# JSybrandt/HypergraphEmbedding

Measured on AMD Instinct MI355X. Metric: training samples/sec + alg-dist SpMV GB/s, HOBE dim=128 at 1/2/4/8 MI355X, higher is better.
Workload: dtype f32; 1 GPU; C3 HG2V_ALG_DIST (HOBE) dim=128, random 100k/50k, 1 step = 1 training epoch; nodes=100000, edges=50000, nnz=1999903, records_per_epoch=59999992, batch=256, dim=128, num_neighbors=5, num_samples=200, parallelism=single GPU

## Files before the change

hypergraphembedding_amd/csrc/hgx_ctx.hip:

```cpp
#include <algorithm>
#include <cstring>
#include <vector>

#include "hgx_internal.h"

int hgx_fail(hgx_ctx *ctx, int code, const char *fmt, ...) {
  if (ctx) {
    char buf[1024];
    va_list ap;
    va_start(ap, fmt);
    vsnprintf(buf, sizeof(buf), fmt, ap);
    va_end(ap);
    ctx->err = buf;
  }
  return code;
}

int hgx_ensure(hgx_ctx *ctx, DevBuf &b, size_t bytes) {
  if (bytes == 0) bytes = 16;
  if (b.bytes >= bytes) return HGX_OK;
  if (b.p) {
    hipFree(b.p);
    b.p = nullptr;
    b.bytes = 0;
// ... 34 lines not shown
    delete ctx;
    return HGX_EHIP;
  }
  ctx->stream = ctx->own_stream;
  hipEventCreate(&ctx->ev0);
  hipEventCreate(&ctx->ev1);
  *out = ctx;
  return HGX_OK;
}

extern "C" int hgx_destroy(hgx_ctx *ctx) {
  if (!ctx) return HGX_OK;
  hipSetDevice(ctx->device);
  hipStreamSynchronize(ctx->stream);
  DevBuf *bufs[] = {&ctx->rp_n, &ctx->col_n, &ctx->rp_e, &ctx->col_e,
                    &ctx->X[0], &ctx->X[1], &ctx->Y[0], &ctx->Y[1], &ctx->mm,
                    &ctx->rp_el, &ctx->col_el, &ctx->blk_n, &ctx->blk_e,
                    &ctx->blk_sn, &ctx->blk_el,
                    &ctx->rec_idx, &ctx->rec_tgt, &ctx->ntab, &ctx->etab,
                    &ctx->nacc, &ctx->eacc, &ctx->s0, &ctx->s1, &ctx->s2,
                    &ctx->s3, &ctx->s4, &ctx->s5, &ctx->s6, &ctx->s7,
                    &ctx->feat_n, &ctx->feat_e, &ctx->cn_p, &ctx->cn_j,
                    &ctx->cn_v, &ctx->ce_p, &ctx->ce_j, &ctx->ce_v,
                    &ctx->hw_n, &ctx->hw_e, &ctx->hw_self, &ctx->bloom_off, &ctx->bloom_bits, &ctx->store,
                    &ctx->st_sel, &ctx->st_keys, &ctx->st_vals, &ctx->st_tmp,
                    &ctx->st_hist};
  for (DevBuf *b : bufs) hgx_release(*b);
  for (LongRows *l : {&ctx->long_n, &ctx->long_e, &ctx->long_sn, &ctx->long_el})
    for (DevBuf *b : {&l->seg, &l->off, &l->rows, &l->part}) hgx_release(*b);
  for (LongRows &l : ctx->long_elr)
    for (DevBuf *b : {&l.seg, &l.off, &l.rows, &l.part}) hgx_release(*b);
  for (hipStream_t &s : ctx->tstream)
    if (s) hipStreamDestroy(s);
  if (ctx->ev0) hipEventDestroy(ctx->ev0);
  if (ctx->ev1) hipEventDestroy(ctx->ev1);
  if (ctx->own_stream) hipStreamDestroy(ctx->own_stream);
  delete ctx;
  return HGX_OK;
}

extern "C" const char *hgx_last_error(const hgx_ctx *ctx) {
  return ctx ? ctx->err.c_str() : "null context";
}

extern "C" int hgx_set_stream(hgx_ctx *ctx, void *hip_stream) {
  if (!ctx) return HGX_EINVAL;
  ctx->stream = hip_stream ? (hipStream_t)hip_stream : ctx->own_stream;
  return HGX_OK;
}

extern "C" int hgx_set_tuning(hgx_ctx *ctx, const char *key, int64_t value) {
  if (!ctx) return HGX_EINVAL;
  HGX_CHECK(ctx, key, HGX_EINVAL, "null tuning key");
  const std::string k(key);
  Tuning &t = ctx->tune;
  if (k == "sample_reject_w") {
    HGX_CHECK(ctx, value >= 0, HGX_EINVAL, "sample_reject_w must be >= 0");
    t.sample_reject_w = value;
  } else if (k == "sample_mode3_shift_e") {
    HGX_CHECK(ctx, value >= -10 && value <= 10, HGX_EINVAL,
              "sample_mode3_shift_e must be in [-10, 10]");
    t.sample_mode3_shift_e = (int)value;
  } else if (k == "sample_mode3_shift") {
    HGX_CHECK(ctx, value >= -10 && value <= 10, HGX_EINVAL,
              "sample_mode3_shift must be in [-10, 10]");
    t.sample_mode3_shift = (int)value;
  } else if (k == "sample_mode3") {
    HGX_CHECK(ctx, value >= 0 && value <= 2, HGX_EINVAL, "sample_mode3 must be 0, 1 or 2");
    t.sample_mode3 = (int)value;
  } else if (k == "train_fused") {
    HGX_CHECK(ctx, value == 0 || value == 1, HGX_EINVAL, "train_fused must be 0 or 1");
    t.train_fused = (int)value;
  } else if (k == "train_lanes") {
    HGX_CHECK(ctx, value == 0 || value == 32 || value == 64, HGX_EINVAL,
              "train_lanes must be 0, 32 or 64");
    t.train_lanes = (int)value;
  } else if (k == "train_tb") {
    HGX_CHECK(ctx, value == 0 || value == 128 || value == 256 || value == 512, HGX_EINVAL,
              "train_tb must be 0, 128, 256 or 512");
    t.train_tb = (int)value;
  } else if (k == "train_wave_pair") {
    HGX_CHECK(ctx, (value >= -1 && value <= 1) || value == 3, HGX_EINVAL,
              "train_wave_pair must be -1, 0, 1 or 3");
    t.train_wave_pair = (int)value;
  } else if (k == "alg_long") {
    HGX_CHECK(ctx, value == 0 || (value >= 64 && value <= (1 << 20)), HGX_EINVAL,
              "alg_long must be 0 or in [64, 2^20]");
    t.alg_long = (int)value;
  } else if (k == "alg_push") {
    HGX_CHECK(ctx, value == 0 || value == 1, HGX_EINVAL, "alg_push must be 0 or 1");
    t.alg_push = (int)value;
  } else if (k == "mlp_fuse_head") {
    HGX_CHECK(ctx, value == 0 || value == 1, HGX_EINVAL, "mlp_fuse_head must be 0 or 1");
    t.mlp_fuse_head = (int)value;
  } else if (k == "mlp_prefetch") {
    HGX_CHECK(ctx, value >= 0 && value <= 2, HGX_EINVAL, "mlp_prefetch must be 0, 1 or 2");
    t.mlp_prefetch = (int)value;
  } else if (k == "mlp_wgrad_split") {
    HGX_CHECK(ctx, value >= 0 && value <= 1, HGX_EINVAL, "mlp_wgrad_split must be 0 or 1");
    t.mlp_wgrad_split = (int)value;
  } else if (k == "svc_lds_m") {
    HGX_CHECK(ctx, value == 64 || value == 128 || value == 192, HGX_EINVAL,
              "svc_lds_m must be 64, 128 or 192");
    t.svc_lds_m = (int)value;
  } else if (k == "ae_chunk_rows") {
    HGX_CHECK(ctx, value >= 0 && value <= (1 << 16), HGX_EINVAL,
              "ae_chunk_rows must be in [0, 65536]");
    t.ae_chunk_rows = (int)value;
  } else if (k == "n2v_expand_w") {
    HGX_CHECK(ctx, value >= 0 && value <= (1 << 20), HGX_EINVAL,
              "n2v_expand_w must be in [0, 2^20]");
    t.n2v_expand_w = (int)value;
  } else if (k == "n2v_chunk_walks") {
    HGX_CHECK(ctx, value >= 0 && value <= (1 << 16), HGX_EINVAL,
              "n2v_chunk_walks must be in [0, 65536]");
    t.n2v_chunk_walks = (int)value;
// ... 200 lines not shown
```

hypergraphembedding_amd/csrc/hgx_internal.h:

```cpp
#pragma once

#include <hip/hip_runtime.h>

#include <cstdarg>
#include <cstdint>
#include <cstdio>
#include <cstdlib>
#include <string>
#include <vector>

#include "hgx.h"

struct DevBuf {
  void *p = nullptr;
  size_t bytes = 0;
  template <class T> T *as() const { return reinterpret_cast<T *>(p); }
};

struct LongRows {
  DevBuf seg;
  DevBuf off;
  DevBuf rows;
  DevBuf part;
  int nlong = 0, nseg = 0, thresh = 0;
// ... 79 lines not shown
  int K = 0;
  DevBuf rec_idx, rec_tgt;
  static constexpr int kMaxRecBlocks = 16;
  int64_t rec_bounds[kMaxRecBlocks + 1] = {0};
  int n_rec_blocks = 0;

  int smp_family = -1;
  uint64_t smp_seed = 0;
  bool rec_in_order = false;

  DevBuf store;
  int64_t n_store = 0, cap_store = 0;
  int store_family = -1, store_K = 0, store_blocks = 0;
  uint64_t store_seed = 0;
  int64_t store_carry = 0;
  std::vector<unsigned> st_hist_host;
  uint64_t st_hist_seed = 0;
  bool st_hist_ok = false;
  DevBuf st_sel, st_keys, st_vals, st_tmp, st_hist;

  int d = 0, dp = 0;
  int64_t node_rows = 0, edge_rows = 0;
  DevBuf ntab, etab, nacc, eacc;
  double train_ms = 0, train_epoch_ms = 0;
  double train_loss_sum = 0;
  int64_t train_records = 0, train_batches = 0;
  int64_t train_fused = 0, train_split = 0;
  int64_t train_multi = 0;
  int train_step_tb = 0, train_step_rpb = 0;

  DevBuf s0, s1, s2, s3, s4, s5, s6, s7;
  hipStream_t tstream[2] = {nullptr, nullptr};
  int tstream_cus = -1;
};

inline int hgx_debug_env(const char *name, int dflt) {
#ifdef HGX_DEBUG_KNOBS
  const char *e = getenv(name);
  return e && e[0] ? atoi(e) : dflt;
#else
  (void)name;
  return dflt;
#endif
}
inline const char *hgx_debug_env_str(const char *name) {
#ifdef HGX_DEBUG_KNOBS
  return getenv(name);
#else
  (void)name;
  return nullptr;
#endif
}

int hgx_fail(hgx_ctx *ctx, int code, const char *fmt, ...);
int hgx_make_row_blocks(hgx_ctx *ctx, const int32_t *rp, int32_t r0, int32_t r1,
                        DevBuf &blk, int &nblk);
int hgx_make_long_rows(hgx_ctx *ctx, const int32_t *rp, int32_t r0, int32_t r1,
                       LongRows &out);
int hgx_ensure(hgx_ctx *ctx, DevBuf &b, size_t bytes);
void hgx_release(DevBuf &b);

#define HGX_HIP(ctx, expr)                                                   \
  do {                                                                       \
    hipError_t e_ = (expr);                                                  \
    if (e_ != hipSuccess)                                                    \
      return hgx_fail((ctx), HGX_EHIP, "%s failed: %s (%s:%d)", #expr,        \
// ... 160 lines not shown
```

hypergraphembedding_amd/csrc/hgx_train.hip:

```cpp
#include <hipcub/hipcub.hpp>

#include <algorithm>
#include <cmath>
#include <cstdlib>
#include <cstring>
#include <vector>

#include "hgx_internal.h"
#include "hgx_train_common.h"
#include "hgx_train_split.h"
#include "hgx_train_step.h"
#include "hgx_train_prep.h"
#include "hgx_train_layout.h"

namespace {

int grid_for(int64_t work, int per_block) {
  int64_t g = (work + per_block - 1) / per_block;
  return (int)std::max<int64_t>(1, std::min<int64_t>(g, 4096));
}

void geometry(int d, int &L, int &VPL) {
  const int nv = (d + 3) / 4;
  L = 1;
// ... 11 lines not shown
using KFn = void (*)(TrainArgs, int);

int env_int(const char *name, int dflt) { return hgx_debug_env(name, dflt); }

template <int L, int VPL, int TB>
KFn fwd_spec(int K, int loss, int act) {
  if (K == 5 && loss == 0 && act == 0) return train_fwd_bwd<L, VPL, 5, true, 1, TB>;
  if (K == 5 && loss == 1 && act == 1) return train_fwd_bwd<L, VPL, 5, true, 2, TB>;
  return nullptr;
}

template <int L, int VPL>
KFn fwd_for(int K, int loss, int act, int tb1) {
  KFn f = tb1 == 512 ? fwd_spec<L, VPL, 512>(K, loss, act)
                     : fwd_spec<L, VPL, kTB>(K, loss, act);
  if (f) return f;
  if (K <= 2) return train_fwd_bwd<L, VPL, 2, false, 0, kTB>;
  if (K <= 5) return train_fwd_bwd<L, VPL, 5, false, 0, kTB>;
  if (K <= 8) return train_fwd_bwd<L, VPL, 8, false, 0, kTB>;
  return train_fwd_bwd<L, VPL, 16, false, 0, kTB>;
}

using KStepFn = void (*)(TrainArgs, int, int, int, int);
using KFlushFn = void (*)(TrainArgs, const int *, const int *, const int *, int, int);

template <int SL, int VW, int TB>
void step_fns(int loss, KStepFn *kf, KFlushFn &kfl) {
  kf[0] = loss == 0 ? train_step<SL, VW, 5, 1, TB, false>
                    : train_step<SL, VW, 5, 2, TB, false>;
  kf[1] = loss == 0 ? train_step<SL, VW, 5, 1, TB, true>
                    : train_step<SL, VW, 5, 2, TB, true>;
  kfl = train_flush<SL * VW / 4>;
}
template <int VW>
void step_fns_pair(int loss, KStepFn *kf, KFlushFn &kfl) {
  kf[0] = loss == 0 ? train_step<64, VW, 5, 1, 512, false, true>
                    : train_step<64, VW, 5, 2, 512, false, true>;
  kf[1] = loss == 0 ? train_step<64, VW, 5, 1, 512, true, true>
                    : train_step<64, VW, 5, 2, 512, true, true>;
  kfl = train_flush<64 * VW / 4>;
}
void step_fns_quad(int loss, KStepFn *kf, KFlushFn &kfl) {
  kf[0] = loss == 0 ? train_step_q<2, 5, 1, false, 2> : train_step_q<2, 5, 2, false, 2>;
  kf[1] = loss == 0 ? train_step_q<2, 5, 1, true, 2> : train_step_q<2, 5, 2, true, 2>;
  kfl = train_flush<32>;
}
constexpr int kPairDefault128 = 3, kPairDefault256 = 1;
bool pick_step(int L, int VPL, int K, int loss, int act, int lanes, int pair, int &sl,
               int &tb, int &rpb, KStepFn *kf, KFlushFn &kfl) {
  if (VPL != 1 || K != 5 || loss != act) return false;
  if (L != 32 && L != 64) return false;
  const int vw = L == 32 && lanes != 32 ? 2 : 4;
  sl = L * 4 / vw;
  const int pair_auto = tb != 0 ? 0 : vw == 2 ? kPairDefault128 : kPairDefault256;
  const int form = pair < 0 ? pair_auto : pair;
  if (sl == 64 && vw == 2 && form == 3) {
    tb = 512;
    rpb = 2;
    step_fns_quad(loss, kf, kfl);
    return true;
  }
  if (sl == 64 && form) {
    tb = 512;
    rpb = 4;
    if (vw == 2) step_fns_pair<2>(loss, kf, kfl);
    else step_fns_pair<4>(loss, kf, kfl);
    return true;
  }
  if (sl == 32) {
    tb = tb == 256 ? 256 : 128;
    if (tb == 128) step_fns<32, 4, 128>(loss, kf, kfl);
    else step_fns<32, 4, 256>(loss, kf, kfl);
  } else if (vw == 2) {
    tb = tb == 512 || tb == 128 ? tb : 256;
    if (tb == 512) step_fns<64, 2, 512>(loss, kf, kfl);
    else if (tb == 128) step_fns<64, 2, 128>(loss, kf, kfl);
    else step_fns<64, 2, 256>(loss, kf, kfl);
  } else {
    tb = 256;
    step_fns<64, 4, 256>(loss, kf, kfl);
  }
  rpb = tb / sl;
  return true;
}

bool pick_kernels(int L, int VPL, int K, int loss, int act, int &tb1, int tb2,
                  KFn &k1, KFn &k2) {
#define HGX_CASE(LL, VV)                                                     \
  if (L == LL && VPL == VV) {                                                \
    k1 = env_int("HGX_TRAIN_GENERIC", 0) == 1                                \
             ? train_fwd_bwd<LL, VV, 16, false, 0, kTB>                      \
             : fwd_for<LL, VV>(K, loss, act, tb1);                           \
// ... 428 lines not shown
      return HGX_OK;
    }
    hipLaunchKernelGGL(shuffle_keys, dim3(grid_for(n, 256)), dim3(256), 0, ctx->stream, seed,
                       ep, n, keys_in, vals_in);
    size_t tmp = sort_tmp;
    if (hipcub::DeviceRadixSort::SortPairs(ctx->s7.as<char>() + sort_off, tmp, keys_in, keys_out,
                                           vals_in, perm, (int)n, 0, 64, ctx->stream) != hipSuccess)
      return hgx_fail(ctx, HGX_EHIP, "shuffle sort failed");
    return HGX_OK;
  }
  int upload(const int64_t *pe) {
    hperm.resize(n);
    for (int64_t i = 0; i < n; i++) {
      if (pe[i] < 0 || pe[i] >= n)
        return hgx_fail(ctx, HGX_EINVAL, "permutation entry out of range");
      hperm[i] = (int)pe[i];
    }
    if (hipMemcpyAsync(perm, hperm.data(), sizeof(int) * n, hipMemcpyHostToDevice,
                       ctx->stream) != hipSuccess ||
        hipStreamSynchronize(ctx->stream) != hipSuccess)
      return hgx_fail(ctx, HGX_EHIP, "permutation upload failed");
    return HGX_OK;
  }
};

struct TrainRun {
  hgx_ctx *ctx;
  const TrainPlan &p;
  TrainArgs ap[2];
  int *skey[2] = {nullptr, nullptr}, *sM[2] = {nullptr, nullptr};
  double *dloss = nullptr, *dpart = nullptr;
  hipStream_t sst, spr;
  std::vector<hipEvent_t> bev, pev;
  int *hbrk = nullptr;
  hipError_t flags_err = hipSuccess;
  int64_t nfused = 0, nsplit = 0, nmulti = 0;
  double batch_ms = 0.0;

  TrainRun(hgx_ctx *c, const TrainPlan &plan) : ctx(c), p(plan), sst(c->stream), spr(c->stream) {}
  ~TrainRun() {
    for (auto e : bev) if (e) (void)hipEventDestroy(e);
    for (auto e : pev) if (e) (void)hipEventDestroy(e);
    if (hbrk) (void)hipHostFree(hbrk);
  }
  int buffers(int *perm) {
    TrainArgs &a = ap[0];
    memset(&a, 0, sizeof(a));
    const size_t s3_bytes = hgx_layout::carve_step(p, {}, a);
    const size_t s5_bytes = hgx_layout::carve_chunk(p, {}, ap, skey, sM);
    HGX_TRY(hgx_ensure(ctx, ctx->s2, sizeof(float) * (size_t)p.SB * p.dp));
    HGX_TRY(hgx_ensure(ctx, ctx->s3, s3_bytes));
    HGX_TRY(hgx_ensure(ctx, ctx->s4, sizeof(float) * (size_t)p.nbatches * p.lstride + 16));
    HGX_TRY(hgx_ensure(ctx, ctx->s5, s5_bytes));
    HGX_TRY(hgx_ensure(ctx, ctx->s6, 64 + sizeof(double) * kLossBlocks));
    HGX_HIP(ctx, hipMemsetAsync(ctx->s5.p, 0, s5_bytes, ctx->stream));
    HGX_HIP(ctx, hipMemsetAsync(ctx->s3.p, 0, s3_bytes, ctx->stream));
    a.idx = ctx->rec_idx.as<int>(), a.tgt = ctx->rec_tgt.as<float>(), a.perm = perm;
    a.n = p.n, a.B = p.batch, a.R = p.R, a.K = p.K, a.dp = p.dp;
    a.ntab = ctx->ntab.as<float>(), a.etab = ctx->etab.as<float>();
    a.nacc = ctx->nacc.as<float>(), a.eacc = ctx->eacc.as<float>();
    a.gslot = ctx->s2.as<float>(), a.lossbuf = ctx->s4.as<float>();
    a.lr = p.lr, a.eps = p.eps, a.loss = p.loss, a.act = p.act;
    a.SB = p.SB, a.nblk1 = p.nblk1, a.lstride = p.lstride;
    a.fused = p.fused ? 1 : 0, a.prpb = p.prpb, a.RW = p.RW, a.MX = p.MX, a.Mmax = p.Mmax;
    hgx_layout::carve_step(p, {ctx->s3.as<char>()}, a);
    hgx_layout::carve_chunk(p, {ctx->s5.as<char>()}, ap, skey, sM);
    dloss = reinterpret_cast<double *>(ctx->s6.as<char>() + 32);
    dpart = reinterpret_cast<double *>(ctx->s6.as<char>() + 64);
    return HGX_OK;
  }
  int init(int *perm) {
    HGX_TRY(buffers(perm));
    if (p.fused)
      HGX_HIP(ctx, hipHostMalloc(reinterpret_cast<void **>(&hbrk),
                                 sizeof(int) * p.CB * (p.overlap ? 2 : 1)));
    if (p.overlap && !p.ahead) {
      HGX_TRY(train_streams(ctx, ctx->tune.train_prep_cus));
      sst = ctx->tstream[0];
      spr = ctx->tstream[1];
    }
    bev.assign(2 * p.nchunks, nullptr);
    pev.assign(p.overlap ? p.nchunks + 1 : 0, nullptr);
    for (auto &e : bev) HGX_HIP(ctx, hipEventCreate(&e));
    for (auto &e : pev) HGX_HIP(ctx, hipEventCreateWithFlags(&e, hipEventDisableTiming));
    return HGX_OK;
  }
  int set_of(int64_t c) const { return p.overlap ? (int)(c & 1) : 0; }

  void begin_epoch() {
    (void)hipMemsetAsync(dloss, 0, sizeof(double), ctx->stream);
    (void)hipMemsetAsync(ap[0].lossbuf, 0, sizeof(float) * (size_t)p.nbatches * p.lstride,
                         ctx->stream);
    if (p.fused) (void)hipMemsetAsync(ap[0].r0acc, 0, hgx_layout::r0acc_bytes(p), ctx->stream);
    if (p.overlap && !p.ahead) {
      (void)hipEventRecord(pev[p.nchunks], ctx->stream);
      (void)hipStreamWaitEvent(sst, pev[p.nchunks], 0);
      (void)hipStreamWaitEvent(spr, pev[p.nchunks], 0);
    }
  }
  void prepare(int64_t c) {
    const int nbc = p.chunk_batches(c), cp = (int)(c & 1), set = set_of(c);
    hipLaunchKernelGGL(train_prep, dim3(p.CB), dim3(kTB), p.prep_smem, spr, ap[0], c * p.CB, nbc,
                       p.P, skey[cp], sM[cp]);
    if (!p.fused) return;
    hipLaunchKernelGGL(train_place, dim3(p.CB), dim3(kTB), p.place_smem, spr, ap[set], nbc, p.CB,
                       skey[cp], sM[cp], skey[cp ^ 1], sM[cp ^ 1], c > 0 ? 1 : 0);
    flags_err = hipMemcpyAsync(hbrk + (size_t)set * p.CB, ap[set].pbrk, sizeof(int) * nbc,
                               hipMemcpyDeviceToHost, spr);
    if (p.overlap) (void)hipEventRecord(pev[c], spr);
  }
  int wait_prepared(int64_t c) {
    hipError_t e = hipSuccess;
    if (p.overlap) {
      e = hipEventSynchronize(pev[c]);
      if (e == hipSuccess && !p.ahead) (void)hipStreamWaitEvent(sst, pev[c], 0);
    } else if (p.fused) {
      e = flags_err != hipSuccess ? flags_err : hipStreamSynchronize(spr);
    }
    if (e == hipSuccess) return HGX_OK;
    return hgx_fail(ctx, HGX_EHIP, "batch preparation failed: %s",
                    hipGetErrorString(hipGetLastError()));
  }
  void run_steps(int64_t c) {
    const int nbc = p.chunk_batches(c), set = set_of(c);
    for (int bi = 0; bi < nbc; bi++) {
      if (!p.fused) {
        hipLaunchKernelGGL(p.k1, dim3(p.nblk1), dim3(p.tb1), 0, sst, ap[0], bi);
        hipLaunchKernelGGL(p.k2, dim3(p.grid2), dim3(p.tb2), 0, sst, ap[0], bi);
        continue;
      }
      const int64_t gbat = c * p.CB + bi;
      const int nrec = (int)std::min<int64_t>(p.batch, p.n - gbat * p.batch);
      const int multi = hbrk[(size_t)set * p.CB + bi] && gbat > 0;
      nmulti += multi;
      hipLaunchKernelGGL(p.kf[multi], dim3(p.NBF), dim3(p.tbf), 0, sst, ap[set], bi, (int)gbat,
                         nrec, (int)gbat);
    }
    (p.fused ? nfused : nsplit) += nbc;
  }
  int run_chunks() {
    if (p.overlap) prepare(0);
    for (int64_t c = 0; c < p.nchunks; c++) {
      if (!p.overlap) prepare(c);
      if (p.ahead && c + 1 < p.nchunks) prepare(c + 1);
      HGX_TRY(wait_prepared(c));
      (void)hipEventRecord(bev[2 * c], sst);
      run_steps(c);
      (void)hipEventRecord(bev[2 * c + 1], sst);
      if (p.overlap && !p.ahead && c + 1 < p.nchunks) {
        if (c >= 1 && hipEventSynchronize(bev[2 * (c - 1) + 1]) != hipSuccess)
          return hgx_fail(ctx, HGX_EHIP, "batch step failed: %s",
                          hipGetErrorString(hipGetLastError()));
        prepare(c + 1);
      }
    }
    return HGX_OK;
  }
  void flush() const {
    const int cp = (int)((p.nchunks - 1) & 1), last_nbc = p.chunk_batches(p.nchunks - 1);
    const int *ml = sM[cp] + (last_nbc - 1);
    const int *mp = last_nbc >= 2 ? sM[cp] + (last_nbc - 2)
                                  : (p.nchunks >= 2 ? sM[cp ^ 1] + (p.CB - 1) : nullptr);
    const int nlast = (int)(p.n - (p.nbatches - 1) * p.batch);
    hipLaunchKernelGGL(p.kfl, dim3(64), dim3(256), 0, sst, ap[0],
                       skey[cp] + (size_t)(last_nbc - 1) * p.Mmax, ml, mp,
                       (int)(p.nbatches - 1), std::min(p.NBF, nlast));
  }
  int finish_epoch(double &lsum) {
    if (p.fused) flush();
    hipLaunchKernelGGL(loss_partial, dim3(kLossBlocks), dim3(kTB), 0, sst, ap[0].lossbuf,
                       p.nbatches * p.lstride, dpart);
    hipLaunchKernelGGL(loss_final, dim3(1), dim3(kLossBlocks), 0, sst, dpart, dloss);
    int ovf = 0;
    if (hipMemcpyAsync(&lsum, dloss, sizeof(double), hipMemcpyDeviceToHost, sst) != hipSuccess ||
        (p.fused && hipMemcpyAsync(&ovf, ap[0].ovf, sizeof(int), hipMemcpyDeviceToHost, sst) !=
                        hipSuccess) ||
        hipStreamSynchronize(sst) != hipSuccess)
      return hgx_fail(ctx, HGX_EHIP, "epoch failed: %s", hipGetErrorString(hipGetLastError()));
    if (ovf)
      return hgx_fail(ctx, HGX_ENUMERIC,
                      "a gradient left the step's fixed-point range (|g| >= %g after "
                      "the 1/batch factor, or NaN): training diverged",
                      (double)kFixLimit);
    for (int64_t c = 0; c < p.nchunks; c++) {
      float m = 0.f;
      if (hipEventElapsedTime(&m, bev[2 * c], bev[2 * c + 1]) == hipSuccess) batch_ms += m;
    }
    return HGX_OK;
  }
  float join() {
    if (p.overlap) {
      (void)hipStreamSynchronize(spr);
      (void)hipStreamSynchronize(sst);
    }
    float ms = 0.f;
    (void)hipEventRecord(ctx->ev1, ctx->stream);
    (void)hipEventSynchronize(ctx->ev1);
    (void)hipEventElapsedTime(&ms, ctx->ev0, ctx->ev1);
    return ms;
  }
  void stats(int epochs, float ms) const {
    ctx->train_ms = batch_ms;
    ctx->train_epoch_ms = ms;
    ctx->train_records = (int64_t)epochs * p.n;
    ctx->train_batches = (int64_t)epochs * p.nbatches;
    ctx->train_fused = nfused;
    ctx->train_split = nsplit;
    ctx->train_multi = nmulti;
    ctx->train_step_tb = p.fused ? p.tbf : 0;
    ctx->train_step_rpb = p.prpb;
  }
};
// ... 78 lines not shown
```

hypergraphembedding_amd/csrc/hgx_train_common.h:

```cpp
#pragma once
#include "hgx_internal.h"

namespace {

constexpr int kTB = 256;
constexpr int kChunkRound = 64;

#ifdef HGX_DEBUG_KNOBS
__constant__ int g_tab = 0;
#else
static constexpr int g_tab = 0;
#endif

#ifdef HGX_DEBUG_KNOBS
__constant__ unsigned long long *g_trace = nullptr;
__constant__ int g_trace_nb = 0;
#else
static constexpr unsigned long long *g_trace = nullptr;
static constexpr int g_trace_nb = 0;
#endif
#define HGX_STAMP(var)                                              \
  do {                                                              \
    if (g_trace) {                                                  \
      asm volatile("s_waitcnt vmcnt(0) lgkmcnt(0)" ::: "memory");   \
// ... 20 lines not shown
  int B, R, K, dp;
  float *ntab, *etab, *nacc, *eacc;
  float *gslot, *gzero, *lossbuf;
  int *bidx;
  float *btgt;
  int *inv, *ukey, *uoff, *ucount;
  int2 *bmeta;
  int SB, nblk1;
  int lstride;
  float lr, eps;
  int loss, act;
  int fused, prpb, RW, MX, Mmax;
  int *pidx, *pbrk;
  unsigned *pcode, *scode;
  float *ptgt;
  int2 *pfo;
  long long *gacc;
  float *shadow;
  long long *r0acc;
  int *ovf;
};

constexpr unsigned kSShared = 0x80000000u;
constexpr unsigned kSOwn = 0x40000000u;
constexpr unsigned kSPend = 0x20000000u;
constexpr unsigned kSLocal = 0x10000000u;
constexpr unsigned kSFirst = 0x08000000u;
constexpr unsigned kFEdge = 0x10000000u;
constexpr int kDefBits = 14;
constexpr unsigned kDefMask = 0xfffu;
constexpr unsigned kSlotMask = 0x3fffu;
constexpr int kFX = 4;
constexpr int kWX = kFX + 2;
constexpr int kPackB = 512;
constexpr int kPrepB = 1366;
constexpr int kSortP = 4096;

__device__ __forceinline__ bool slot_is_edge(int s, int K) {
  return s == 1 || s == 3 || s >= 4 + K;
}

__device__ __forceinline__ float act_f(int act, float z) {
  return act == 0 ? 1.0f / (1.0f + expf(-z)) : (z > 0.f ? z : 0.f);
}
__device__ __forceinline__ float act_d(int act, float z, float y) {
  return act == 0 ? y * (1.0f - y) : (z > 0.f ? 1.f : 0.f);
}
__device__ __forceinline__ void head_loss(int loss, float y, float yt,
                                          float &lv, float &g) {
  const float eps = 1e-7f;
  if (loss == 0) {
    const float ytc = fminf(fmaxf(yt, eps), 1.f);
    const float ypc = fminf(fmaxf(y, eps), 1.f);
    lv = ytc * logf(ytc / ypc);
    g = (y >= eps && y <= 1.f) ? -ytc / ypc : 0.f;
  } else {
    const float df = y - yt;
    lv = df * df;
    g = 2.f * df;
  }
}

__device__ __forceinline__ float4 f4(float a) { return make_float4(a, a, a, a); }
__device__ __forceinline__ float4 operator+(float4 a, float4 b) {
  return make_float4(a.x + b.x, a.y + b.y, a.z + b.z, a.w + b.w);
}
// ... 23 lines not shown
```

hypergraphembedding_amd/csrc/hgx_train_prep.h:

```cpp
#pragma once
#include <rocprim/block/block_radix_sort.hpp>

#include "hgx_train_step.h"

namespace {

__device__ int block_exclusive_scan(int v, int *total, int *s_ws) {
  const int lane = threadIdx.x & 63, wave = threadIdx.x >> 6;
  int inc = v;
#pragma unroll
  for (int off = 1; off < 64; off <<= 1) {
    const int o = __shfl_up(inc, off);
    if (lane >= off) inc += o;
  }
  if (lane == 63) s_ws[wave] = inc;
  __syncthreads();
  int base = 0, tot = 0;
  for (int w = 0; w < kTB / 64; w++) {
    if (w < wave) base += s_ws[w];
    tot += s_ws[w];
  }
  __syncthreads();
  *total = tot;
  return base + inc - v;
// ... 214 lines not shown
  const int G = (a.B + RPB - 1) / RPB * RPB;
  const int *prev = nullptr;
  int Mp = 0, Mpp = 0;
  if (cb > 0) {
    prev = skey_cur + (size_t)(cb - 1) * a.Mmax;
    Mp = sM_cur[cb - 1];
  } else if (has_prev) {
    prev = skey_pc + (size_t)(CB - 1) * a.Mmax;
    Mp = sM_pc[CB - 1];
  }
  if (cb > 1) Mpp = sM_cur[cb - 2];
  else if (has_prev) Mpp = sM_pc[CB - 2 + cb];
  const int U = a.ucount[cb];
  int *s_prev = s_dyn, *s_u = s_dyn + a.Mmax;
  __shared__ int s_brk;
  if (threadIdx.x == 0) s_brk = 0;
  for (int j = threadIdx.x; j < Mp; j += kTB) s_prev[j] = prev[j];
  for (int j = threadIdx.x; j < U; j += kTB) s_u[j] = a.ukey[(size_t)cb * SB + j];
  const int *bidx = a.bidx + (size_t)cb * a.B * R;
  const float *btgt = a.btgt + (size_t)cb * a.B * 3;
  __syncthreads();
  for (int i = threadIdx.x; i < nb && Mp; i += kTB) {
    int e0 = -1;
    for (int s2 = 0; s2 < R; s2++) {
      const int row = bidx[i * R + s2];
      if (row == 0) continue;
      const int j = bsearch_lds(s_prev, Mp, ((int)slot_is_edge(s2, K) << 30) | row);
      if (j < 0) continue;
      if (e0 >= 0 && j != e0) s_brk = 1;
      e0 = j;
    }
  }
  __syncthreads();
  if (threadIdx.x == 0) a.pbrk[cb] = s_brk;
  {
    const int per = (nb + kTB - 1) / kTB, i0 = threadIdx.x * per, i1 = min(i0 + per, nb);
    int cs = 0;
    for (int i = i0; i < i1; i++) {
      int any = 0;
      for (int s = 4; s < R; s++) any |= bidx[i * R + s];
      s_pos[i] = any;
      cs += any == 0;
    }
    int NS = 0;
    int bs = block_exclusive_scan(cs, &NS, s_ws);
    const int NBF = G / RPB;
    for (int i = i0; i < i1; i++) {
      const bool sh = s_pos[i] == 0;
      const int p = sh ? bs : NS + (i - bs);
      s_pos[i] = (p % NBF) * RPB + p / NBF;
      bs += sh;
    }
  }
  int *pidx = a.pidx + (size_t)cb * G * RW;
  unsigned *pcode = a.pcode + (size_t)cb * G * RW;
  float *ptgt = a.ptgt + (size_t)cb * G * 3;
  for (int t = threadIdx.x; t < G * RW; t += kTB) {
    pidx[t] = 0;
    pcode[t] = 0u;
  }
  for (int t = threadIdx.x; t < G * 3; t += kTB) ptgt[t] = 0.f;
  __syncthreads();
  const unsigned *sc = a.scode + (size_t)cb * SB;
  for (int t = threadIdx.x; t < nb * R; t += kTB) {
    const int i = t / R, s = t - i * R;
    const int row = bidx[t];
    unsigned code = 0;
// ... 277 lines not shown
```

hypergraphembedding_amd/csrc/hgx_train_step.h:

```cpp
#pragma once
#include "hgx_train_split.h"

namespace {



constexpr double kFixScale = 17592186044416.0;
constexpr double kFixInv = 1.0 / 17592186044416.0;
constexpr float kFixLimit = 32.f;

__device__ __forceinline__ unsigned long long to_fix(float v) {
  return (unsigned long long)__double2ll_rn((double)v * kFixScale);
}
__device__ __forceinline__ float from_fix(long long v) {
  return (float)((double)v * kFixInv);
}
__device__ __forceinline__ float act_d_nc(int act, float z, float y) {
  return act == 0 ? mul_nc(y, sub_nc(1.0f, y)) : (z > 0.f ? 1.f : 0.f);
}
__device__ __forceinline__ void head_loss_nc(int loss, float y, float yt,
                                             float &lv, float &g) {
  const float eps = 1e-7f;
  if (loss == 0) {
    const float ytc = fminf(fmaxf(yt, eps), 1.f);
    const float ypc = fminf(fmaxf(y, eps), 1.f);
    lv = mul_nc(ytc, logf(ytc / ypc));
    g = (y >= eps && y <= 1.f) ? -ytc / ypc : 0.f;
  } else {
    const float df = sub_nc(y, yt);
    lv = mul_nc(df, df);
    g = 2.f * df;
  }
}

template <int VW>
struct SV;
template <>
struct SV<4> {
  using T = float4;
  struct Fx {
    longlong2 a, b;
  };
  static __device__ __forceinline__ T zero() { return f4(0.f); }
  static __device__ __forceinline__ T add(T x, T y) { return x + y; }
  static __device__ __forceinline__ T mul(T x, float m) {
    return make_float4(x.x * m, x.y * m, x.z * m, x.w * m);
  }
  static __device__ __forceinline__ T fma(float s, T v, T c) { return fma4(s, v, c); }
  static __device__ __forceinline__ float dot(T x, T y) { return dot4(x, y); }
  static __device__ __forceinline__ void adagrad(T &p, T &ac, T g, float lr, float eps) {
    adagrad4_hw(p, ac, g, lr, eps);
  }
  static __device__ __forceinline__ void pin(T &v) {
    asm volatile("" : "+v"(v.x), "+v"(v.y), "+v"(v.z), "+v"(v.w));
  }
  static __device__ __forceinline__ Fx ldfix(const long long *e, int lane) {
    const longlong2 *g = reinterpret_cast<const longlong2 *>(e) + 2 * lane;
    return {g[0], g[1]};
  }
  static __device__ __forceinline__ T unfix(const Fx &g) {
    return make_float4(from_fix(g.a.x), from_fix(g.a.y), from_fix(g.b.x), from_fix(g.b.y));
  }
  static __device__ __forceinline__ void addfix(long long *e, int lane, T v, int &bad) {
    bad |= !(fabsf(v.x) < kFixLimit) | !(fabsf(v.y) < kFixLimit) |
           !(fabsf(v.z) < kFixLimit) | !(fabsf(v.w) < kFixLimit);
    unsigned long long *d = reinterpret_cast<unsigned long long *>(e) + 4 * lane;
    atomicAdd(d + 0, to_fix(v.x));
    atomicAdd(d + 1, to_fix(v.y));
    atomicAdd(d + 2, to_fix(v.z));
    atomicAdd(d + 3, to_fix(v.w));
  }
  static __device__ __forceinline__ void zerofix(long long *e, int lane) {
    longlong2 *g = reinterpret_cast<longlong2 *>(e) + 2 * lane;
    g[0] = g[1] = make_longlong2(0, 0);
  }
  static __device__ __forceinline__ Fx fxadd(const Fx &x, const Fx &y) {
    return {make_longlong2(x.a.x + y.a.x, x.a.y + y.a.y),
            make_longlong2(x.b.x + y.b.x, x.b.y + y.b.y)};
  }
  static __device__ __forceinline__ Fx fxzero() {
    return {make_longlong2(0, 0), make_longlong2(0, 0)};
  }
};
template <>
struct SV<2> {
  using T = float2;
  struct Fx {
    longlong2 a;
  };
  static __device__ __forceinline__ T zero() { return make_float2(0.f, 0.f); }
  static __device__ __forceinline__ T add(T x, T y) { return make_float2(x.x + y.x, x.y + y.y); }
  static __device__ __forceinline__ T mul(T x, float m) { return make_float2(x.x * m, x.y * m); }
  static __device__ __forceinline__ T fma(float s, T v, T c) {
    return make_float2(fmaf(s, v.x, c.x), fmaf(s, v.y, c.y));
  }
  static __device__ __forceinline__ float dot(T x, T y) {
    return add_nc(mul_nc(x.x, y.x), mul_nc(x.y, y.y));
  }
  static __device__ __forceinline__ void adagrad(T &p, T &ac, T g, float lr, float eps) {
    const float *gv = &g.x;
    float *pp = &p.x, *aa = &ac.x;
#pragma unroll
    for (int c = 0; c < 2; c++) {
      const float na = add_nc(aa[c], mul_nc(gv[c], gv[c]));
      aa[c] = na;
      const float den = add_nc(__builtin_amdgcn_sqrtf(na), eps);
      pp[c] = sub_nc(pp[c], mul_nc(mul_nc(lr, gv[c]), __builtin_amdgcn_rcpf(den)));
    }
  }
  static __device__ __forceinline__ void pin(T &v) { asm volatile("" : "+v"(v.x), "+v"(v.y)); }
  static __device__ __forceinline__ Fx ldfix(const long long *e, int lane) {
    return {reinterpret_cast<const longlong2 *>(e)[lane]};
  }
  static __device__ __forceinline__ T unfix(const Fx &g) {
    return make_float2(from_fix(g.a.x), from_fix(g.a.y));
  }
  static __device__ __forceinline__ void addfix(long long *e, int lane, T v, int &bad) {
    bad |= !(fabsf(v.x) < kFixLimit) | !(fabsf(v.y) < kFixLimit);
    unsigned long long *d = reinterpret_cast<unsigned long long *>(e) + 2 * lane;
    atomicAdd(d + 0, to_fix(v.x));
    atomicAdd(d + 1, to_fix(v.y));
  }
  static __device__ __forceinline__ void zerofix(long long *e, int lane) {
    reinterpret_cast<longlong2 *>(e)[lane] = make_longlong2(0, 0);
  }
  static __device__ __forceinline__ Fx fxadd(const Fx &x, const Fx &y) {
    return {make_longlong2(x.a.x + y.a.x, x.a.y + y.a.y)};
  }
  static __device__ __forceinline__ Fx fxzero() { return {make_longlong2(0, 0)}; }
};
template <int VW>
__device__ __forceinline__ void fold(typename SV<VW>::T &p, typename SV<VW>::T &ac,
                                     const typename SV<VW>::Fx &g, float lr, float eps) {
  SV<VW>::adagrad(p, ac, SV<VW>::unfix(g), lr, eps);
}

template <int L, int VW>
__device__ __forceinline__ typename SV<VW>::T *sh_row(const TrainArgs &a, int par, int m,
                                                      int which) {
  return reinterpret_cast<typename SV<VW>::T *>(a.shadow) +
         (((size_t)par * a.MX + m) * 2 + which) * L;
}
template <int L, int VW>
__device__ __forceinline__ long long *gacc_row(const TrainArgs &a, int par, int m) {
  return a.gacc + ((size_t)par * a.MX + m) * (VW * L);
}
template <int L, int VW>
__device__ __forceinline__ typename SV<VW>::T *tab_row(const TrainArgs &a, bool edge, int acc,
                                                       int row) {
  float *t = acc ? (edge ? a.eacc : a.nacc) : (edge ? a.etab : a.ntab);
  return reinterpret_cast<typename SV<VW>::T *>(t) + (size_t)row * L;
}

__device__ __forceinline__ void st_row(float2 *p, float2 v) {
// ... 44 lines not shown
}
template <int L, int VW>
struct Row0Loads {
  static constexpr int NC = 2 * L;
  typename SV<VW>::Fx g[R0S<VW * L>::n];
  typename SV<VW>::T rp, ra;
};
template <int L, int VW>
__device__ __forceinline__ void row0_issue(const TrainArgs &a, int q,
                                           Row0Loads<L, VW> &ld) {
  using RL = Row0Loads<L, VW>;
  const int col = threadIdx.x % RL::NC;
  const int tab = col / L, c = col % L, ppar = (q + 2) % 3;
  ld.rp = (q ? sh_row<L, VW>(a, ppar, tab, 0) : tab_row<L, VW>(a, tab, 0, 0))[c];
  ld.ra = (q ? sh_row<L, VW>(a, ppar, tab, 1) : tab_row<L, VW>(a, tab, 1, 0))[c];
#pragma unroll
  for (int j = 0; j < R0S<VW * L>::n; j++)
    ld.g[j] = SV<VW>::ldfix(r0_row<L, VW>(a, ppar, j, tab), c);
}
template <int L, int VW>
__device__ __forceinline__ void row0_finish(const TrainArgs &a, int q,
                                            const Row0Loads<L, VW> &ld,
                                            typename SV<VW>::T &p0, typename SV<VW>::T &a0) {
  using S = SV<VW>;
  typename S::Fx t = ld.g[0];
#pragma unroll
  for (int j = 1; j < R0S<VW * L>::n; j++) t = S::fxadd(t, ld.g[j]);
  if (g_tab & 2048) t = S::fxzero();
  if (q) S::adagrad(p0, a0, S::unfix(t), a.lr, a.eps);
}

#ifndef HGX_TRAIN_R0EARLY
#define HGX_TRAIN_R0EARLY 1
#endif

template <int VW, int K, int MODE, bool MULTI>
__device__ __forceinline__ void train_step_pair(const TrainArgs &a, int cb, int gb, int nb,
                                                int q) {
  constexpr int L = 64, RPB = 4, NW = 2 * RPB, TB = NW * L, R = 4 + 2 * K, J = 2 + K;
  constexpr int NZ = 1 + K;
  using S = SV<VW>;
  using V = typename S::T;
  static_assert(R + kWX <= 32, "slot and batch words fit the first 32 lanes");
  static_assert(NZ % 2 == 0, "the head dots reduce in groups of four, then two");
  constexpr bool kR0E = HGX_TRAIN_R0EARLY && VW == 2;
  __shared__ V s_z[2][RPB][L];
  __shared__ V s_gl[RPB][R][L];
  __shared__ V s_r0[2][L];
  __shared__ float s_loss[RPB];
  __shared__ float s_x[RPB][4];
  unsigned long long ts[8] = {0, 0, 0, 0, 0, 0, 0, 0};
  if (g_trace) ts[0] = __builtin_amdgcn_s_memrealtime();
  const int wave = __builtin_amdgcn_readfirstlane(threadIdx.x / L), lane = threadIdx.x % L;
  const int grp = wave >> 1, half = wave & 1;
  const bool edge = half;
  const int NBF = gridDim.x, RW = a.RW;
  const int par = q % 3, ppar = (q + 2) % 3, zpar = (q + 1) % 3;
  const size_t gi = ((size_t)cb * NBF + blockIdx.x) * RPB + grp;
  const int *ri = a.pidx + gi * RW;
  const unsigned *rc = a.pcode + gi * RW;
  const float *yt = a.ptgt + gi * 3;
  const int sl = lane < RW ? lane : 0;
  const int rv = ri[sl];
  const int cv = (int)rc[sl];
  const int tv = __float_as_int(yt[lane < 3 ? lane : 0]);
  Row0Loads<L, VW> r0l;
// ... 73 lines not shown
      st_row(&Tw[(size_t)frow[0] * L + lane], fp);
      st_row(&Aw[(size_t)frow[0] * L + lane], fa);
    }
    unsigned pm = 0;
#pragma unroll
    for (int j = 0; j < J; j++)
      if (code[j] & kSPend) pm |= 1u << j;
    if (!has) pm = 0;
    auto fold_pass = [&]() {
      if (pm == 0) return;
      const int ps = __builtin_ctz(pm);
      unsigned cd = 0;
#pragma unroll
      for (int j = 0; j < J; j++)
        if (j == ps) cd = code[j];
      const unsigned mp = (cd >> kDefBits) & kDefMask;
      const typename S::Fx gg = S::ldfix(gacc_row<L, VW>(a, ppar, mp), lane);
      V pp = sh_row<L, VW>(a, ppar, mp, 0)[lane], aa = sh_row<L, VW>(a, ppar, mp, 1)[lane];
      unsigned wm = 0;
#pragma unroll
      for (int j = 0; j < J; j++)
        if (((code[j] >> kDefBits) & kDefMask) == mp) wm |= 1u << j;
      wm &= pm;
      fold<VW>(pp, aa, gg, a.lr, a.eps);
#pragma unroll
      for (int j = 0; j < J; j++)
        if ((wm >> j) & 1u) {
          Pv[j] = pp;
          Av[j] = aa;
        }
      pm &= ~wm;
    };
    fold_pass();
    if (MULTI) {
      fold_pass();
      if (pm != 0) {
#pragma unroll
        for (int j = 0; j < J; j++) {
          if (!((pm >> j) & 1u)) continue;
          const int mp = (code[j] >> kDefBits) & kDefMask;
          const typename S::Fx gg = S::ldfix(gacc_row<L, VW>(a, ppar, mp), lane);
          V pp = sh_row<L, VW>(a, ppar, mp, 0)[lane], aa = sh_row<L, VW>(a, ppar, mp, 1)[lane];
          fold<VW>(pp, aa, gg, a.lr, a.eps);
          Pv[j] = pp;
          Av[j] = aa;
        }
      }
    }
    const int act = MODE == 1 ? 0 : 1;
    const int lossk = MODE == 1 ? 0 : 1;
    float zh = 0.f, yh = 0.f, zk[K], sk[K];
    if (has) {
#pragma unroll
      for (int j = 0; j < J; j++)
        if (row[j] == 0) Pv[j] = s_r0[half][lane];
      float zz[NZ];
      zz[0] = S::dot(Pv[0], Pv[1]);
#pragma unroll
      for (int k = 0; k < K; k++) zz[1 + k] = S::dot(Pv[2 + k], Pv[0]);
      hgx::wave_allreduce_sum_n<NZ>(zz);
      zh = zz[0];
      yh = act_f(act, zh);
      float PQ = 0.f;
#pragma unroll
      for (int k = 0; k < K; k++) {
        zk[k] = zz[1 + k];
        sk[k] = act_f(act, zk[k]);
// ... 259 lines not shown
    const int lossk = MODE == 1 ? 0 : 1;
    by_role([&](auto rl) __attribute__((always_inline)) {
      using QR = QRole<decltype(rl)::value, J, JH>;
      constexpr int ROLE = decltype(rl)::value;
      unsigned pm = 0;
#pragma unroll
      for (int j = 0; j < J; j++)
        if (((QR::pm >> j) & 1u) && (code[j] & kSPend)) pm |= 1u << j;
      auto fold_pass = [&]() __attribute__((always_inline)) {
        if (pm == 0) return;
        const int ps = __builtin_ctz(pm);
        unsigned cd = 0;
#pragma unroll
        for (int j = 0; j < J; j++)
          if (j == ps) cd = code[j];
        const unsigned mp = (cd >> kDefBits) & kDefMask;
        const typename S::Fx gg = S::ldfix(gacc_row<L, VW>(a, ppar, mp), lane);
        V pp = sh_row<L, VW>(a, ppar, mp, 0)[lane], aa = sh_row<L, VW>(a, ppar, mp, 1)[lane];
        unsigned wm = 0;
#pragma unroll
        for (int j = 0; j < J; j++)
          if (((code[j] >> kDefBits) & kDefMask) == mp) wm |= 1u << j;
        wm &= pm;
        fold<VW>(pp, aa, gg, a.lr, a.eps);
#pragma unroll
        for (int j = 0; j < J; j++)
          if (((QR::pm >> j) & 1u) && ((wm >> j) & 1u)) {
            Pv[j] = pp;
            Av[j] = aa;
          }
        pm &= ~wm;
      };
      fold_pass();
      if (MULTI) {
        fold_pass();
        if (pm != 0) {
#pragma unroll
          for (int j = 0; j < J; j++) {
            if (!((QR::pm >> j) & 1u) || !((pm >> j) & 1u)) continue;
            const int mp = (code[j] >> kDefBits) & kDefMask;
            const typename S::Fx gg = S::ldfix(gacc_row<L, VW>(a, ppar, mp), lane);
            V pp = sh_row<L, VW>(a, ppar, mp, 0)[lane], aa = sh_row<L, VW>(a, ppar, mp, 1)[lane];
            fold<VW>(pp, aa, gg, a.lr, a.eps);
            Pv[j] = pp;
            Av[j] = aa;
          }
        }
      }
#pragma unroll
      for (int j = 0; j < J; j++)
        if (((QR::pm >> j) & 1u) && row[j] == 0) Pv[j] = s_r0[half][lane];
      constexpr int K0 = ROLE == kQList ? KH : 0, K1 = ROLE == kQHead ? KH : K;
      constexpr int Z0 = ROLE == kQList ? 0 : 1, NQ = Z0 + K1 - K0;
      float zz[NQ];
      if (Z0) zz[0] = S::dot(Pv[0], Pv[1]);
#pragma unroll
      for (int k = K0; k < K1; k++) zz[Z0 + k - K0] = S::dot(Pv[2 + k], Pv[0]);
      hgx::wave_allreduce_sum_n<NQ>(zz);
      if (lane == 0) {
        if (Z0) s_zx[grp][half][0] = zz[0];
#pragma unroll
        for (int k = K0; k < K1; k++) s_zx[grp][half][1 + k] = zz[Z0 + k - K0];
      }
      if (ROLE == kQList) {
#pragma unroll
        for (int k = KH; k < K; k++) s_t[grp][half][k - KH][lane] = Pv[2 + k];
      }
// ... 529 lines not shown
```

Baseline: 43.79 million records/s.

## Merge single/multi step kernels to drop per-chunk host flag sync; add quad RPB=1 default

When the fused step uses the same kernel for both the single and multi-parent cases, the per-chunk device-to-host copy of break flags and the host stream synchronize are skipped, and every batch launches the MULTI variant. The multi-parent fold pass now runs only when unresolved parents remain, so the generic path stays cheap. The multi-batch count moves into a device atomic that is read back with the overflow flag. The dim=128 default switches to a new quad form with 1 row per block at 256 threads. A magic-number double-to-fixed conversion is added for VW=4, and the pinned flag buffer is cached in the context. The trade-off is always running the multi-capable kernel, with some extra branch work, in exchange for removing host round trips.

Measured after the change: 45.92 million records/s, median of 6. +4.9%, better.

```diff
diff --git a/hypergraphembedding_amd/csrc/hgx_ctx.hip b/hypergraphembedding_amd/csrc/hgx_ctx.hip
--- a/hypergraphembedding_amd/csrc/hgx_ctx.hip
+++ b/hypergraphembedding_amd/csrc/hgx_ctx.hip
@@ -90,6 +90,7 @@
     for (DevBuf *b : {&l.seg, &l.off, &l.rows, &l.part}) hgx_release(*b);
   for (hipStream_t &s : ctx->tstream)
     if (s) hipStreamDestroy(s);
+  if (ctx->train_hbrk) hipHostFree(ctx->train_hbrk);
   if (ctx->ev0) hipEventDestroy(ctx->ev0);
   if (ctx->ev1) hipEventDestroy(ctx->ev1);
   if (ctx->own_stream) hipStreamDestroy(ctx->own_stream);
@@ -138,8 +139,8 @@
               "train_tb must be 0, 128, 256 or 512");
     t.train_tb = (int)value;
   } else if (k == "train_wave_pair") {
-    HGX_CHECK(ctx, (value >= -1 && value <= 1) || value == 3, HGX_EINVAL,
-              "train_wave_pair must be -1, 0, 1 or 3");
+    HGX_CHECK(ctx, (value >= -1 && value <= 1) || value == 3 || value == 4, HGX_EINVAL,
+              "train_wave_pair must be -1, 0, 1, 3 or 4");
     t.train_wave_pair = (int)value;
   } else if (k == "alg_long") {
     HGX_CHECK(ctx, value == 0 || (value >= 64 && value <= (1 << 20)), HGX_EINVAL,
diff --git a/hypergraphembedding_amd/csrc/hgx_fix.h b/hypergraphembedding_amd/csrc/hgx_fix.h
--- /dev/null
+++ b/hypergraphembedding_amd/csrc/hgx_fix.h
@@ -0,0 +1,34 @@
+#pragma once
+
+#if defined(__HIPCC__) || defined(__CUDACC__)
+#define HGX_FIX_HD __host__ __device__ __forceinline__
+#else
+#define HGX_FIX_HD inline
+#endif
+
+constexpr double kFixScale = 17592186044416.0;
+constexpr double kFixInv = 1.0 / 17592186044416.0;
+constexpr float kFixLimit = 32.f;
+
+#ifndef HGX_TRAIN_FIXMAGIC
+#define HGX_TRAIN_FIXMAGIC 1
+#endif
+
+HGX_FIX_HD unsigned long long to_fix_magic(float v) {
+  constexpr double kMagic = 6755399441055744.0;
+  const double y = (double)v * kFixScale + kMagic;
+  return __builtin_bit_cast(unsigned long long, y) -
+         __builtin_bit_cast(unsigned long long, kMagic);
+}
+HGX_FIX_HD unsigned long long to_fix_rn(float v) {
+#if defined(__HIP_DEVICE_COMPILE__)
+  return (unsigned long long)__double2ll_rn((double)v * kFixScale);
+#else
+  return (unsigned long long)__builtin_llrint((double)v * kFixScale);
+#endif
+}
+template <int VW>
+HGX_FIX_HD unsigned long long to_fix(float v) {
+  return HGX_TRAIN_FIXMAGIC == 2 || (HGX_TRAIN_FIXMAGIC == 1 && VW == 4) ? to_fix_magic(v)
+                                                                         : to_fix_rn(v);
+}
diff --git a/hypergraphembedding_amd/csrc/hgx_internal.h b/hypergraphembedding_amd/csrc/hgx_internal.h
--- a/hypergraphembedding_amd/csrc/hgx_internal.h
+++ b/hypergraphembedding_amd/csrc/hgx_internal.h
@@ -135,6 +135,8 @@
   DevBuf s0, s1, s2, s3, s4, s5, s6, s7;
   hipStream_t tstream[2] = {nullptr, nullptr};
   int tstream_cus = -1;
+  int *train_hbrk = nullptr;
+  size_t train_hbrk_n = 0;
 };
 
 inline int hgx_debug_env(const char *name, int dflt) {
diff --git a/hypergraphembedding_amd/csrc/hgx_train.hip b/hypergraphembedding_amd/csrc/hgx_train.hip
--- a/hypergraphembedding_amd/csrc/hgx_train.hip
+++ b/hypergraphembedding_amd/csrc/hgx_train.hip
@@ -67,20 +67,27 @@
                     : train_step<SL, VW, 5, 2, TB, true>;
   kfl = train_flush<SL * VW / 4>;
 }
+#ifndef HGX_TRAIN_CHUNKWAIT
+#define HGX_TRAIN_CHUNKWAIT 0
+#endif
+constexpr bool kMergePair4 = HGX_TRAIN_ONEKERNEL >= 1;
+constexpr bool kMergeAll = HGX_TRAIN_ONEKERNEL == 2;
 template <int VW>
 void step_fns_pair(int loss, KStepFn *kf, KFlushFn &kfl) {
-  kf[0] = loss == 0 ? train_step<64, VW, 5, 1, 512, false, true>
-                    : train_step<64, VW, 5, 2, 512, false, true>;
+  constexpr bool M0 = kMergeAll || (kMergePair4 && VW == 4);
+  kf[0] = loss == 0 ? train_step<64, VW, 5, 1, 512, M0, true>
+                    : train_step<64, VW, 5, 2, 512, M0, true>;
   kf[1] = loss == 0 ? train_step<64, VW, 5, 1, 512, true, true>
                     : train_step<64, VW, 5, 2, 512, true, true>;
   kfl = train_flush<64 * VW / 4>;
 }
+template <int RPB>
 void step_fns_quad(int loss, KStepFn *kf, KFlushFn &kfl) {
-  kf[0] = loss == 0 ? train_step_q<2, 5, 1, false, 2> : train_step_q<2, 5, 2, false, 2>;
-  kf[1] = loss == 0 ? train_step_q<2, 5, 1, true, 2> : train_step_q<2, 5, 2, true, 2>;
+  kf[0] = loss == 0 ? train_step_q<2, 5, 1, kMergeAll, RPB> : train_step_q<2, 5, 2, kMergeAll, RPB>;
+  kf[1] = loss == 0 ? train_step_q<2, 5, 1, true, RPB> : train_step_q<2, 5, 2, true, RPB>;
   kfl = train_flush<32>;
 }
-constexpr int kPairDefault128 = 3, kPairDefault256 = 1;
+constexpr int kPairDefault128 = 4, kPairDefault256 = 1;
 bool pick_step(int L, int VPL, int K, int loss, int act, int lanes, int pair, int &sl,
                int &tb, int &rpb, KStepFn *kf, KFlushFn &kfl) {
   if (VPL != 1 || K != 5 || loss != act) return false;
@@ -92,7 +99,13 @@
   if (sl == 64 && vw == 2 && form == 3) {
     tb = 512;
     rpb = 2;
-    step_fns_quad(loss, kf, kfl);
+    step_fns_quad<2>(loss, kf, kfl);
+    return true;
+  }
+  if (sl == 64 && vw == 2 && form == 4) {
+    tb = 256;
+    rpb = 1;
+    step_fns_quad<1>(loss, kf, kfl);
     return true;
   }
   if (sl == 64 && form) {
@@ -587,16 +600,18 @@
   double *dloss = nullptr, *dpart = nullptr;
   hipStream_t sst, spr;
   std::vector<hipEvent_t> bev, pev;
+  const bool merged;
   int *hbrk = nullptr;
   hipError_t flags_err = hipSuccess;
   int64_t nfused = 0, nsplit = 0, nmulti = 0;
   double batch_ms = 0.0;
 
-  TrainRun(hgx_ctx *c, const TrainPlan &plan) : ctx(c), p(plan), sst(c->stream), spr(c->stream) {}
+  TrainRun(hgx_ctx *c, const TrainPlan &plan)
+      : ctx(c), p(plan), sst(c->stream), spr(c->stream),
+        merged(plan.fused && plan.kf[0] == plan.kf[1] && !HGX_TRAIN_CHUNKWAIT) {}
   ~TrainRun() {
     for (auto e : bev) if (e) (void)hipEventDestroy(e);
     for (auto e : pev) if (e) (void)hipEventDestroy(e);
-    if (hbrk) (void)hipHostFree(hbrk);
   }
   int buffers(int *perm) {
     TrainArgs &a = ap[0];
@@ -626,9 +641,17 @@
   }
   int init(int *perm) {
     HGX_TRY(buffers(perm));
-    if (p.fused)
-      HGX_HIP(ctx, hipHostMalloc(reinterpret_cast<void **>(&hbrk),
-                                 sizeof(int) * p.CB * (p.overlap ? 2 : 1)));
+    if (p.fused && !merged) {
+      const size_t need = (size_t)p.CB * (p.overlap ? 2 : 1);
+      if (ctx->train_hbrk_n < need) {
+        if (ctx->train_hbrk) (void)hipHostFree(ctx->train_hbrk);
+        ctx->train_hbrk = nullptr, ctx->train_hbrk_n = 0;
+        HGX_HIP(ctx, hipHostMalloc(reinterpret_cast<void **>(&ctx->train_hbrk),
+                                   sizeof(int) * need));
+        ctx->train_hbrk_n = need;
+      }
+      hbrk = ctx->train_hbrk;
+    }
     if (p.overlap && !p.ahead) {
       HGX_TRY(train_streams(ctx, ctx->tune.train_prep_cus));
       sst = ctx->tstream[0];
@@ -660,8 +683,9 @@
     if (!p.fused) return;
     hipLaunchKernelGGL(train_place, dim3(p.CB), dim3(kTB), p.place_smem, spr, ap[set], nbc, p.CB,
                        skey[cp], sM[cp], skey[cp ^ 1], sM[cp ^ 1], c > 0 ? 1 : 0);
-    flags_err = hipMemcpyAsync(hbrk + (size_t)set * p.CB, ap[set].pbrk, sizeof(int) * nbc,
-                               hipMemcpyDeviceToHost, spr);
+    if (!merged)
+      flags_err = hipMemcpyAsync(hbrk + (size_t)set * p.CB, ap[set].pbrk, sizeof(int) * nbc,
+                                 hipMemcpyDeviceToHost, spr);
     if (p.overlap) (void)hipEventRecord(pev[c], spr);
   }
   int wait_prepared(int64_t c) {
@@ -669,7 +693,7 @@
     if (p.overlap) {
       e = hipEventSynchronize(pev[c]);
       if (e == hipSuccess && !p.ahead) (void)hipStreamWaitEvent(sst, pev[c], 0);
-    } else if (p.fused) {
+    } else if (p.fused && !merged) {
       e = flags_err != hipSuccess ? flags_err : hipStreamSynchronize(spr);
     }
     if (e == hipSuccess) return HGX_OK;
@@ -686,8 +710,7 @@
       }
       const int64_t gbat = c * p.CB + bi;
       const int nrec = (int)std::min<int64_t>(p.batch, p.n - gbat * p.batch);
-      const int multi = hbrk[(size_t)set * p.CB + bi] && gbat > 0;
-      nmulti += multi;
+      const int multi = merged || (hbrk[(size_t)set * p.CB + bi] && gbat > 0);
       hipLaunchKernelGGL(p.kf[multi], dim3(p.NBF), dim3(p.tbf), 0, sst, ap[set], bi, (int)gbat,
                          nrec, (int)gbat);
     }
@@ -726,13 +749,15 @@
     hipLaunchKernelGGL(loss_partial, dim3(kLossBlocks), dim3(kTB), 0, sst, ap[0].lossbuf,
                        p.nbatches * p.lstride, dpart);
     hipLaunchKernelGGL(loss_final, dim3(1), dim3(kLossBlocks), 0, sst, dpart, dloss);
-    int ovf = 0;
+    int fl[2] = {0, 0};
+    static_assert(kOvfMulti == 1, "read with the range flag");
     if (hipMemcpyAsync(&lsum, dloss, sizeof(double), hipMemcpyDeviceToHost, sst) != hipSuccess ||
-        (p.fused && hipMemcpyAsync(&ovf, ap[0].ovf, sizeof(int), hipMemcpyDeviceToHost, sst) !=
+        (p.fused && hipMemcpyAsync(fl, ap[0].ovf, sizeof(fl), hipMemcpyDeviceToHost, sst) !=
                         hipSuccess) ||
         hipStreamSynchronize(sst) != hipSuccess)
       return hgx_fail(ctx, HGX_EHIP, "epoch failed: %s", hipGetErrorString(hipGetLastError()));
-    if (ovf)
+    nmulti = fl[1];
+    if (fl[0])
       return hgx_fail(ctx, HGX_ENUMERIC,
                       "a gradient left the step's fixed-point range (|g| >= %g after "
                       "the 1/batch factor, or NaN): training diverged",
diff --git a/hypergraphembedding_amd/csrc/hgx_train_common.h b/hypergraphembedding_amd/csrc/hgx_train_common.h
--- a/hypergraphembedding_amd/csrc/hgx_train_common.h
+++ b/hypergraphembedding_amd/csrc/hgx_train_common.h
@@ -76,6 +76,7 @@
 constexpr unsigned kSlotMask = 0x3fffu;
 constexpr int kFX = 4;
 constexpr int kWX = kFX + 2;
+constexpr int kOvfMulti = 1;
 constexpr int kPackB = 512;
 constexpr int kPrepB = 1366;
 constexpr int kSortP = 4096;
diff --git a/hypergraphembedding_amd/csrc/hgx_train_prep.h b/hypergraphembedding_amd/csrc/hgx_train_prep.h
--- a/hypergraphembedding_amd/csrc/hgx_train_prep.h
+++ b/hypergraphembedding_amd/csrc/hgx_train_prep.h
@@ -270,7 +270,10 @@
     }
   }
   __syncthreads();
-  if (threadIdx.x == 0) a.pbrk[cb] = s_brk;
+  if (threadIdx.x == 0) {
+    a.pbrk[cb] = s_brk;
+    if (s_brk) atomicAdd(a.ovf + kOvfMulti, 1);
+  }
   {
     const int per = (nb + kTB - 1) / kTB, i0 = threadIdx.x * per, i1 = min(i0 + per, nb);
     int cs = 0;
diff --git a/hypergraphembedding_amd/csrc/hgx_train_step.h b/hypergraphembedding_amd/csrc/hgx_train_step.h
--- a/hypergraphembedding_amd/csrc/hgx_train_step.h
+++ b/hypergraphembedding_amd/csrc/hgx_train_step.h
@@ -1,17 +1,11 @@
 #pragma once
+#include "hgx_fix.h"
 #include "hgx_train_split.h"
 
 namespace {
 
 
 
-constexpr double kFixScale = 17592186044416.0;
-constexpr double kFixInv = 1.0 / 17592186044416.0;
-constexpr float kFixLimit = 32.f;
-
-__device__ __forceinline__ unsigned long long to_fix(float v) {
-  return (unsigned long long)__double2ll_rn((double)v * kFixScale);
-}
 __device__ __forceinline__ float from_fix(long long v) {
   return (float)((double)v * kFixInv);
 }
@@ -65,10 +59,10 @@
     bad |= !(fabsf(v.x) < kFixLimit) | !(fabsf(v.y) < kFixLimit) |
            !(fabsf(v.z) < kFixLimit) | !(fabsf(v.w) < kFixLimit);
     unsigned long long *d = reinterpret_cast<unsigned long long *>(e) + 4 * lane;
-    atomicAdd(d + 0, to_fix(v.x));
-    atomicAdd(d + 1, to_fix(v.y));
-    atomicAdd(d + 2, to_fix(v.z));
-    atomicAdd(d + 3, to_fix(v.w));
+    atomicAdd(d + 0, to_fix<4>(v.x));
+    atomicAdd(d + 1, to_fix<4>(v.y));
+    atomicAdd(d + 2, to_fix<4>(v.z));
+    atomicAdd(d + 3, to_fix<4>(v.w));
   }
   static __device__ __forceinline__ void zerofix(long long *e, int lane) {
     longlong2 *g = reinterpret_cast<longlong2 *>(e) + 2 * lane;
@@ -118,8 +112,8 @@
   static __device__ __forceinline__ void addfix(long long *e, int lane, T v, int &bad) {
     bad |= !(fabsf(v.x) < kFixLimit) | !(fabsf(v.y) < kFixLimit);
     unsigned long long *d = reinterpret_cast<unsigned long long *>(e) + 2 * lane;
-    atomicAdd(d + 0, to_fix(v.x));
-    atomicAdd(d + 1, to_fix(v.y));
+    atomicAdd(d + 0, to_fix<2>(v.x));
+    atomicAdd(d + 1, to_fix<2>(v.y));
   }
   static __device__ __forceinline__ void zerofix(long long *e, int lane) {
     reinterpret_cast<longlong2 *>(e)[lane] = make_longlong2(0, 0);
@@ -230,6 +224,10 @@
 
 #ifndef HGX_TRAIN_R0EARLY
 #define HGX_TRAIN_R0EARLY 1
+#endif
+
+#ifndef HGX_TRAIN_ONEKERNEL
+#define HGX_TRAIN_ONEKERNEL 1
 #endif
 
 template <int VW, int K, int MODE, bool MULTI>
@@ -369,7 +367,7 @@
       pm &= ~wm;
     };
     fold_pass();
-    if (MULTI) {
+    if (MULTI && pm != 0) {
       fold_pass();
       if (pm != 0) {
 #pragma unroll
@@ -695,7 +693,7 @@
         pm &= ~wm;
       };
       fold_pass();
-      if (MULTI) {
+      if (MULTI && pm != 0) {
         fold_pass();
         if (pm != 0) {
 #pragma unroll
```
